# barlettacarmen/CrCNN

Hardware: AMD Instinct MI355X
Metric: encrypted images/sec (higher is better)
Workload: dtype u64

## Files before the change

crcnn_amd/csrc/kernels_mfma1.hip:

```cpp
#include "kernels.h"
#include "limbred.h"
#include "boxstage.h"
#include <cstdlib>

typedef int v4i __attribute__((ext_vector_type(4)));
typedef signed char i8;
#define NPL 7
#define MAXK 8

struct Conv1Args {
    const i8 *xr; const i8 *wl; u64 *ys; i8 *xl_out; const ModParams *mods; const u64 *bias;
    int n, k, B, Bout, b0, xd, yo, xs, ystr, P, F, mtiles;
    unsigned img_stride, plane_bytes, poly_bytes;
    unsigned out_img_bytes;
    int out_zdc;
    int narrow;
    int acc0[MAXK][13];
    u32 qbits[MAXK], qfold[MAXK];
    unsigned px_rs;
    int px_taps, px_yf, px_pair;
    int acc7[MAXK][7];
};

__device__ __forceinline__ void limb_digits1(u64 r, u64 q, int (&d)[NPL])
{
    long long v = r > (q >> 1) ? (long long)r - (long long)q : (long long)r;
#pragma unroll
    for (int l = 0; l < NPL; l++) { d[l] = (int)(signed char)(v & 0xff); v = (v - d[l]) >> 8; }
}

__device__ __forceinline__ void conv1_store4(const Conv1Args &a, i8 *stage, const long long (&cv)[4], int mm, int f0, int chan_bytes, u64 q, int slot, int b)
{
    if (mm >= 2 * a.P) return;
    if (a.xl_out) {
        if (f0 >= chan_bytes) return;
        u32 lo[4], hi[4];
#pragma unroll
        for (int reg = 0; reg < 4; reg++) { const u64 dg = f0 + reg < a.F ? centred_digit_bytes(cv[reg]) : 0; lo[reg] = (u32)dg;
            hi[reg] = (u32)(dg >> 32); }
        const u32 t0 = __builtin_amdgcn_perm(lo[1], lo[0], 0x05010400u), t1 = __builtin_amdgcn_perm(lo[1], lo[0], 0x07030602u);
        const u32 u0 = __builtin_amdgcn_perm(lo[3], lo[2], 0x05010400u), u1 = __builtin_amdgcn_perm(lo[3], lo[2], 0x07030602u);
        const u32 t2 = __builtin_amdgcn_perm(hi[1], hi[0], 0x05010400u), t3 = __builtin_amdgcn_perm(hi[1], hi[0], 0x07030602u);
        const u32 u2 = __builtin_amdgcn_perm(hi[3], hi[2], 0x05010400u), u3 = __builtin_amdgcn_perm(hi[3], hi[2], 0x07030602u);
        u32 pl[NPL];
        pl[0] = __builtin_amdgcn_perm(u0, t0, 0x05040100u); pl[1] = __builtin_amdgcn_perm(u0, t0, 0x07060302u);
        pl[2] = __builtin_amdgcn_perm(u1, t1, 0x05040100u); pl[3] = __builtin_amdgcn_perm(u1, t1, 0x07060302u);
        pl[4] = __builtin_amdgcn_perm(u2, t2, 0x05040100u); pl[5] = __builtin_amdgcn_perm(u2, t2, 0x07060302u);
        pl[6] = __builtin_amdgcn_perm(u3, t3, 0x05040100u);
        i8 *sp; unsigned pstride;
        if (a.out_zdc) { sp = stage + ((mm & 1) * a.P + (mm >> 1)) * a.out_zdc + f0; pstride = 2 * a.P * a.out_zdc; }
        else { sp = stage + mm * (NPL * 32) + f0; pstride = 32; }
#pragma unroll
        for (int l = 0; l < NPL; l++) *reinterpret_cast<u32 *>(sp + l * pstride) = pl[l];
    } else {
#pragma unroll
        for (int reg = 0; reg < 4; reg++)
            if (f0 + reg < a.F) a.ys[(((size_t)slot * a.B + b) * a.F + f0 + reg) * (2 * a.P) + mm] = (u64)(cv[reg] + ((cv[reg] >> 63) & (long long)q));
    }
}
__device__ __forceinline__ void conv1_copy_out(const Conv1Args &a, const i8 *stage, int slot, int b)
{
    i8 *dst = a.xl_out + ((size_t)slot * a.Bout + a.b0 + b) * a.out_img_bytes;
    if (a.out_zdc) {
        for (unsigned o = threadIdx.x; o < a.out_img_bytes / 16; o += blockDim.x)
            *reinterpret_cast<uint4 *>(dst + (size_t)o * 16) = *reinterpret_cast<const uint4 *>(stage + (size_t)o * 16);
    } else {
        const unsigned per_plane = a.out_img_bytes / (NPL * 16);
        for (unsigned o = threadIdx.x; o < NPL * per_plane; o += blockDim.x) {
            const unsigned l = o / per_plane, rem = o - l * per_plane;
            *reinterpret_cast<uint4 *>(dst + (size_t)o * 16) = *reinterpret_cast<const uint4 *>(stage + (rem >> 1) * (NPL * 32) + l * 32 +
                (rem & 1) * 16);
        }
    }
}

__global__ void __launch_bounds__(768) mfma_conv1_kernel(Conv1Args a)
{
    extern __shared__ __attribute__((aligned(16))) i8 lds[];
    const int lane = threadIdx.x & 63, wave = __builtin_amdgcn_readfirstlane(threadIdx.x >> 6), nwaves = blockDim.x >> 6;
    const int slot = blockIdx.x, i = slot / a.n, s = slot % a.n;
    const u64 q = a.mods[i].q;
    const u32 qbits = a.qbits[i], qfold = a.qfold[i];
    const int g = lane >> 4, r16 = lane & 15;
    const bool narrow = a.narrow != 0;
    const int nt = narrow ? (wave >> 2) & 1 : wave & 1;
    const int tile0 = !narrow ? wave >> 1 : nt ? wave - 4 : (wave < 4 ? wave : wave - 4), tile_step = !narrow ? nwaves >> 1 : nt ? 4 : nwaves - 4;
    const bool nar = narrow && nt;
    v4i wv[NPL];
    {
        const i8 *ws = a.wl + (size_t)slot * (NPL * 32 * 64) + (nt * 16 + r16) * 64 + g * 16;
        if (!nar) {
#pragma unroll
            for (int l = 0; l < NPL; l++) wv[l] = *reinterpret_cast<const v4i *>(ws + l * (32 * 64));
        } else {
            const i8 *wp = a.wl + (size_t)slot * (NPL * 32 * 64) + (16 + (r16 >> 2)) * 64 + g * 16;
#pragma unroll
            for (int grp = 0; grp < 2; grp++) {
                const int pl = 4 * grp + (r16 & 3);
                wv[grp] = pl < NPL ? *reinterpret_cast<const v4i *>(wp + pl * (32 * 64)) : v4i{0, 0, 0, 0};
            }
#pragma unroll
            for (int l = 2; l < NPL; l++) wv[l] = v4i{0, 0, 0, 0};
        }
    }
    u32 PB[7];
#pragma unroll
    for (int j = 0; j < 6; j++) PB[j] = (u32)a.acc0[i][2 * j] + ((u32)a.acc0[i][2 * j + 1] << 8);
    PB[6] = (u32)a.acc0[i][12];
    const u32 rcp_yo = (65536u + (u32)a.yo - 1) / (u32)a.yo;
    const int f0 = nt * 16 + 4 * g;
    long long bvc[4];
#pragma unroll
    for (int reg = 0; reg < 4; reg++) {
        const int f = f0 + reg;
        const u64 bv = (a.bias && f < a.F && !(lane & 1)) ? a.bias[((size_t)f * a.k + i) * a.n + s] : 0;
        bvc[reg] = bv > (q >> 1) ? (long long)(bv - q) : (long long)bv;
    }
    long long bvn = 0;
    if (nar) {
        const int f = 16 + g;
        const u64 bv = (a.bias && f < a.F && !(lane & 1)) ? a.bias[((size_t)f * a.k + i) * a.n + s] : 0;
        bvn = bv > (q >> 1) ? (long long)(bv - q) : (long long)bv;
    }
    i8 *stage = lds + 2 * (size_t)a.img_stride;
    const i8 *ximg = a.xr + (size_t)slot * a.B * a.img_stride;
    const int pieces = a.img_stride / 1024;
    auto issue_img = [&](int b) {
        i8 *dst = lds + (b & 1) * (size_t)a.img_stride;
        const i8 *src = ximg + (size_t)b * a.img_stride + lane * 16;
        for (int pc = wave; pc < pieces; pc += nwaves)
            __builtin_amdgcn_global_load_lds((const __attribute__((address_space(1))) void *)(src + pc * 1024),
                (__attribute__((address_space(3))) void *)(dst + pc * 1024), 16, 0, 0);
    };
    if (a.xl_out && a.out_zdc && threadIdx.x < 16) { const unsigned e = a.out_img_bytes - 16 + threadIdx.x;
        if (e >= (unsigned)(NPL * 2 * a.P * a.out_zdc)) stage[e] = 0; }
    issue_img(0);
    const int chan_bytes = a.out_zdc ? a.out_zdc : 32;
    for (int b = 0; b < a.B; b++) {
        __builtin_amdgcn_s_waitcnt(0 | (7 << 4) | (15 << 8));
        __syncthreads();
        if (b + 1 < a.B) issue_img(b + 1);
        const i8 *img = lds + (b & 1) * (size_t)a.img_stride;
        for (int mt = tile0; mt < a.mtiles; mt += tile_step) {
            v4i acc[13];
#pragma unroll
            for (int d = 0; d < 13; d++) acc[d] = v4i{0, 0, 0, 0};
            const int mm = mt * 16 + r16, mrow = min(mm, 2 * a.P - 1), p = mrow >> 1, c = mrow & 1, ox = (int)(((u32)p * rcp_yo) >> 16), oy = p - ox * a.yo;
            const int r0 = min(ox * a.xs + 2 * g, a.xd - 1), r1 = min(ox * a.xs + 2 * g + 1, a.xd - 1);
            const int off = oy * a.ystr, sh = off & 3;
            const i8 *p0 = img + c * a.poly_bytes + (off & ~3) + r0 * 32, *p1 = img + c * a.poly_bytes + (off & ~3) + r1 * 32;
            auto window = [&](int l) {
                const u32 *q0 = reinterpret_cast<const u32 *>(p0 + l * a.plane_bytes), *q1 = reinterpret_cast<const u32 *>(p1 + l * a.plane_bytes);
                const u32 a0 = q0[0], a1 = q0[1], a2 = q0[2], b0 = q1[0], b1 = q1[1], b2 = q1[2];
                return v4i{(int)__builtin_amdgcn_alignbyte(a1, a0, sh), (int)__builtin_amdgcn_alignbyte(a2, a1, sh), (int)__builtin_amdgcn_alignbyte(b1, b0,
                    sh),
                           (int)__builtin_amdgcn_alignbyte(b2, b1, sh)};
            };
            if (nar) {
                v4i hi6;
#pragma unroll
                for (int l = 0; l < NPL; l++) {
                    const v4i av = window(l);
                    acc[l] = __builtin_amdgcn_mfma_i32_16x16x64_i8(wv[0], av, v4i{0, 0, 0, 0}, 0, 0, 0);
                    if (l < 6) acc[7 + l] = __builtin_amdgcn_mfma_i32_16x16x64_i8(wv[1], av, v4i{0, 0, 0, 0}, 0, 0, 0);
                    else hi6 = __builtin_amdgcn_mfma_i32_16x16x64_i8(wv[1], av, v4i{0, 0, 0, 0}, 0, 0, 0);
                }
                int D[13];
#pragma unroll
                for (int d = 0; d < 13; d++) {
                    int sum = 0;
#pragma unroll
                    for (int l = 0; l < NPL; l++) {
                        const int m = d - l;
                        if (m < 0 || m >= NPL) continue;
                        sum += m < 4 ? acc[l][m] : (l < 6 ? acc[7 + l][m - 4] : hi6[m - 4]);
                    }
                    D[d] = sum;
                }
                const long long cvn = diag_fold_short_centred(D, q, qbits, qfold, bvn, PB);
                const int f = 16 + g;
                if (mm >= 2 * a.P) continue;
                if (a.xl_out) {
                    if (f >= chan_bytes) continue;
                    const u64 dg = f < a.F ? centred_digit_bytes(cvn) : 0;
                    i8 *sp; unsigned pstride;
                    if (a.out_zdc) { sp = stage + ((mm & 1) * a.P + (mm >> 1)) * a.out_zdc + f; pstride = 2 * a.P * a.out_zdc; }
                    else { sp = stage + mm * (NPL * 32) + f; pstride = 32; }
#pragma unroll
                    for (int l = 0; l < NPL; l++) sp[l * pstride] = (i8)(dg >> (8 * l));
                } else if (f < a.F) a.ys[(((size_t)slot * a.B + b) * a.F + f) * (2 * a.P) + mm] = (u64)(cvn + ((cvn >> 63) & (long long)q));
                continue;
            }
#pragma unroll
            for (int l = 0; l < NPL; l++) {
                const v4i av = window(l);
#pragma unroll
                for (int m2 = 0; m2 < NPL; m2++)
                    acc[l + m2] = __builtin_amdgcn_mfma_i32_16x16x64_i8(wv[m2], av, acc[l + m2], 0, 0, 0);
            }
            long long cv[4];
#pragma unroll
            for (int reg = 0; reg < 4; reg++) {
                int D[13];
#pragma unroll
                for (int d = 0; d < 13; d++) D[d] = acc[d][reg];
                cv[reg] = diag_fold_short_centred(D, q, qbits, qfold, bvc[reg], PB);
            }
            conv1_store4(a, stage, cv, mm, f0, chan_bytes, q, slot, b);
        }
        if (a.xl_out) {
            __syncthreads();
            conv1_copy_out(a, stage, slot, b);
        }
    }
}

#define NJ 5
__global__ void __launch_bounds__(512) mfma_conv1_kernel_px(Conv1Args a)
{
    extern __shared__ __attribute__((aligned(16))) i8 lds[];
    const int lane = threadIdx.x & 63, wave = __builtin_amdgcn_readfirstlane(threadIdx.x >> 6), nwaves = blockDim.x >> 6;
    const int slot = blockIdx.x, i = slot / a.n, s = slot % a.n;
    const u64 q = a.mods[i].q;
    const u32 qbits = a.qbits[i], qfold = a.qfold[i];
    const int g = lane >> 4, r16 = lane & 15, nt = wave & 1, tile0 = wave >> 1, tile_step = nwaves >> 1;
    v4i wv[NPL][NJ];
    {
        const i8 *ws = a.wl + (size_t)slot * (NPL * NJ * 32 * 64) + (nt * 16 + r16) * 64 + g * 16;
#pragma unroll
        for (int m = 0; m < NPL; m++)
#pragma unroll
            for (int j = 0; j < NJ; j++) wv[m][j] = *reinterpret_cast<const v4i *>(ws + (m * NJ + j) * (32 * 64));
    }
    u32 PB[4];
#pragma unroll
    for (int j = 0; j < 3; j++) PB[j] = (u32)a.acc7[i][2 * j] + ((u32)a.acc7[i][2 * j + 1] << 8);
    PB[3] = (u32)a.acc7[i][6];
    u32 toff[NJ];
#pragma unroll
    for (int j = 0; j < NJ; j++) {
        const int last = a.px_pair ? a.px_taps - 2 : a.px_taps - 1;
        const int t0 = min(2 * (4 * j + g), last), t1 = min(2 * (4 * j + g) + 1, a.px_taps - 1);
        const u32 o0 = (u32)(t0 / a.px_yf) * a.px_rs + (u32)(t0 % a.px_yf) * 8, o1 = (u32)(t1 / a.px_yf) * a.px_rs + (u32)(t1 % a.px_yf) * 8;
        toff[j] = o0 | (o1 << 16);
    }
    const u32 rcp_yo = (65536u + (u32)a.yo - 1) / (u32)a.yo;
    const int f0 = nt * 16 + 4 * g;
    long long bvc[4];
#pragma unroll
    for (int reg = 0; reg < 4; reg++) {
        const int f = f0 + reg;
        const u64 bv = (a.bias && f < a.F && !(lane & 1)) ? a.bias[((size_t)f * a.k + i) * a.n + s] : 0;
        bvc[reg] = bv > (q >> 1) ? (long long)(bv - q) : (long long)bv;
    }
    i8 *stage = lds + 2 * (size_t)a.img_stride;
    const i8 *ximg = a.xr + (size_t)slot * a.B * a.img_stride;
    const int pieces = a.img_stride / 1024;
    auto issue_img = [&](int b) {
        i8 *dst = lds + (b & 1) * (size_t)a.img_stride;
        const i8 *src = ximg + (size_t)b * a.img_stride + lane * 16;
        for (int pc = wave; pc < pieces; pc += nwaves)
            __builtin_amdgcn_global_load_lds((const __attribute__((address_space(1))) void *)(src + pc * 1024),
                (__attribute__((address_space(3))) void *)(dst + pc * 1024), 16, 0, 0);
    };
    if (a.xl_out && a.out_zdc && threadIdx.x < 16) { const unsigned e = a.out_img_bytes - 16 + threadIdx.x;
        if (e >= (unsigned)(NPL * 2 * a.P * a.out_zdc)) stage[e] = 0; }
    issue_img(0);
    const int chan_bytes = a.out_zdc ? a.out_zdc : 32;
    for (int b = 0; b < a.B; b++) {
        __builtin_amdgcn_s_waitcnt(0 | (7 << 4) | (15 << 8));
        __syncthreads();
        if (b + 1 < a.B) issue_img(b + 1);
        const i8 *img = lds + (b & 1) * (size_t)a.img_stride;
        for (int mt = tile0; mt < a.mtiles; mt += tile_step) {
            const int mm = mt * 16 + r16, mrow = min(mm, 2 * a.P - 1), p = mrow >> 1, c = mrow & 1, ox = (int)(((u32)p * rcp_yo) >> 16), oy = p - ox * a.yo;
            const i8 *win = img + c * a.poly_bytes + (u32)(ox * a.xs) * a.px_rs + (u32)(oy * a.ystr) * 8;
            v4i bv[NJ];
            if (a.px_pair) {
#pragma unroll
                for (int j = 0; j < NJ; j++) bv[j] = *reinterpret_cast<const v4i *>(win + (toff[j] & 0xffffu));
            } else {
#pragma unroll
                for (int j = 0; j < NJ; j++) {
                    const uint2 t0 = *reinterpret_cast<const uint2 *>(win + (toff[j] & 0xffffu)), t1 = *reinterpret_cast<const uint2 *>(win + (toff[j] >> 16));
                    bv[j] = v4i{(int)t0.x, (int)t0.y, (int)t1.x, (int)t1.y};
                }
            }
            v4i acc[NPL];
#pragma unroll
            for (int m = 0; m < NPL; m++) acc[m] = __builtin_amdgcn_mfma_i32_16x16x64_i8(wv[m][0], bv[0], v4i{0, 0, 0, 0}, 0, 0, 0);
#pragma unroll
            for (int j = 1; j < NJ; j++)
#pragma unroll
                for (int m = 0; m < NPL; m++) acc[m] = __builtin_amdgcn_mfma_i32_16x16x64_i8(wv[m][j], bv[j], acc[m], 0, 0, 0);
            long long cv[4];
#pragma unroll
            for (int reg = 0; reg < 4; reg++) {
                int E[NPL];
#pragma unroll
                for (int m = 0; m < NPL; m++) E[m] = acc[m][reg];
                cv[reg] = diag7_fold_centred(E, q, qbits, qfold, bvc[reg], PB);
            }
            conv1_store4(a, stage, cv, mm, f0, chan_bytes, q, slot, b);
        }
        if (a.xl_out) {
            __syncthreads();
            conv1_copy_out(a, stage, slot, b);
        }
    }
}

#define RG 4
#define RSL 32
__global__ void __launch_bounds__(256) limb_pack_rows1_kernel(const u64 *x, i8 *xr, const ModParams *mods, int n, int k, int B, int xd, int yd, int packed,
                                                              unsigned img_stride, unsigned plane_bytes, unsigned poly_bytes)
{
    __shared__ __attribute__((aligned(16))) i8 st[RSL * NPL * RG * 32];
    const int sblocks = n / RSL;
    const int sb = blockIdx.x % (sblocks * k), i = sb / sblocks, s0 = (sb % sblocks) * RSL;
    const int rgs = (xd + RG - 1) / RG;
    size_t r = blockIdx.x / (sblocks * k);
    const int rg = (int)(r % rgs); r /= rgs; const int c = (int)(r % 2); const int b = (int)(r / 2);
    const u64 q = mods[i].q;
    const int lane = threadIdx.x & (RSL - 1), qrow = (threadIdx.x >> 5) & (RG - 1), h = threadIdx.x >> 7, row = rg * RG + qrow;
    {
        u32 pl[NPL][4];
#pragma unroll
        for (int l = 0; l < NPL; l++)
#pragma unroll
            for (int wv = 0; wv < 4; wv++) pl[l][wv] = 0;
        if (row < xd) {
            const u64 *src = x + ((((size_t)b * xd * yd + (size_t)row * yd + h * 16) * 2 + c) * k + i) * (size_t)n + s0 + lane;
#pragma unroll
            for (int colx = 0; colx < 16; colx++)
                if (h * 16 + colx < yd) {
                    u64 v = src[(size_t)colx * 2 * k * n];
                    if (packed) v = (v & 0xffffffffULL) | ((v >> 32) << 28);
                    const u64 dg = balanced_digit_bytes(v, q);
#pragma unroll
                    for (int l = 0; l < NPL; l++) pl[l][colx >> 2] |= (u32)((dg >> (8 * l)) & 0xff) << (8 * (colx & 3));
                }
        }
        i8 *sp = st + (size_t)lane * (NPL * RG * 32) + qrow * 32 + h * 16;
#pragma unroll
        for (int l = 0; l < NPL; l++) *reinterpret_cast<uint4 *>(sp + l * (RG * 32)) = make_uint4(pl[l][0], pl[l][1], pl[l][2], pl[l][3]);
    }
    __syncthreads();
    const int pieces_per_run = RG * 2, rows_here = min(RG, xd - rg * RG);
    for (int o = threadIdx.x; o < RSL * NPL * pieces_per_run; o += 256) {
        const int run = o / pieces_per_run, part = o - run * pieces_per_run, sl = run / NPL, l = run - sl * NPL;
        if ((part >> 1) >= rows_here) continue;
        i8 *dst = xr + (((size_t)i * n + s0 + sl) * B + b) * img_stride + (size_t)l * plane_bytes + (size_t)c * poly_bytes + (size_t)(rg * RG) * 32 + part * 16;
        *reinterpret_cast<uint4 *>(dst) = *reinterpret_cast<const uint4 *>(st + (size_t)run * (RG * 32) + part * 16);
    }
}
template <bool BOX>
__global__ void __launch_bounds__(256) limb_pack_rows1_kernel_px(const u64 *x, i8 *xr, const ModParams *mods, int n, int k, int B, int xd, int yd, int packed,
                                                                 unsigned img_stride, unsigned poly_bytes, unsigned rs, int xdo, int ydo, int bxf, int byf, int xs,
                                                                 int ys)
{
    extern __shared__ __attribute__((aligned(16))) i8 stp[];
    const unsigned sstride = RG * rs + 16;
    const int sblocks = n / RSL;
    const int sb = blockIdx.x % (sblocks * k), i = sb / sblocks, s0 = (sb % sblocks) * RSL;
    const int rgs = (xdo + RG - 1) / RG;
    size_t r = blockIdx.x / (sblocks * k);
    const int rg = (int)(r % rgs); r /= rgs; const int c = (int)(r % 2); const int b = (int)(r / 2);
    const u64 q = mods[i].q;
    const int lane = threadIdx.x & (RSL - 1), qrow = (threadIdx.x >> 5) & (RG - 1), h = threadIdx.x >> 7, row = rg * RG + qrow;
    if (row < xdo) {
        const size_t cs = (size_t)2 * k * n;
        const u64 *src = x + ((((size_t)b * xd * yd + (size_t)row * yd + h * 16) * 2 + c) * k + i) * (size_t)n + s0 + lane;
        u64 *sp = reinterpret_cast<u64 *>(stp + (size_t)lane * sstride + qrow * rs) + h * 16;
        if constexpr (!BOX) {
#pragma unroll
            for (int colx = 0; colx < 16; colx++) {
                const int col = h * 16 + colx;
                if ((unsigned)col * 8 >= rs) continue;
                u64 dg = 0;
                if (col < yd) {
                    u64 v = src[(size_t)colx * cs];
                    if (packed) v = (v & 0xffffffffULL) | ((v >> 32) << 28);
                    dg = balanced_digit_bytes(v, q);
                }
                sp[colx] = dg;
            }
        } else {
            u64 sum[16];
#pragma unroll
            for (int colx = 0; colx < 16; colx++) sum[colx] = 0;
            for (int a = 0; a < bxf; a++)
                for (int bb = 0; bb < byf; bb++) {
                    const u64 *tp = src + ((size_t)a * xs * yd + (size_t)bb * ys) * cs;
#pragma unroll
                    for (int colx = 0; colx < 16; colx++)
                        if (h * 16 + colx < ydo) {
                            u64 v = tp[(size_t)colx * cs];
                            if (packed) v = (v & 0xffffffffULL) | ((v >> 32) << 28);
                            sum[colx] += v;
                        }
                }
#pragma unroll
            for (int colx = 0; colx < 16; colx++) {
                const int col = h * 16 + colx;
                if ((unsigned)col * 8 >= rs) continue;
                sp[colx] = col < ydo ? balanced_digit_bytes(sum_reduce16(sum[colx], q), q) : 0;
            }
        }
    }
    __syncthreads();
    const int per_run = RG * rs / 16, valid = min(RG, xdo - rg * RG) * (int)rs / 16;
    for (int o = threadIdx.x; o < RSL * per_run; o += 256) {
        const int sl = o / per_run, part = o - sl * per_run;
        if (part >= valid) continue;
        i8 *dst = xr + (((size_t)i * n + s0 + sl) * B + b) * img_stride + (size_t)c * poly_bytes + (size_t)(rg * RG) * rs + part * 16;
        *reinterpret_cast<uint4 *>(dst) = *reinterpret_cast<const uint4 *>(stp + (size_t)sl * sstride + part * 16);
    }
}
#define BOX_LD 16
static_assert(BOX_RG == RG && BOX_RSL == RSL, "boxstage.h describes this pack's workgroup");
__global__ void __launch_bounds__(256) limb_pack_box_kernel_px(const u64 *x, i8 *xr, const ModParams *mods, int n, int k, int B, int xd, int yd, int packed,
                                                               unsigned img_stride, unsigned poly_bytes, unsigned rs, int xdo, int ydo, int bxf, int byf, int xs,
                                                               int ys)
{
    extern __shared__ __attribute__((aligned(16))) i8 stp[];
    u64 *ring = reinterpret_cast<u64 *>(stp);
    i8 *dig = stp + box_ring_bytes(yd, bxf, xs);
    const unsigned sstride = RG * rs + 16;
    const int sblocks = n / RSL;
    const int sb = blockIdx.x % (sblocks * k), i = sb / sblocks, s0 = (sb % sblocks) * RSL;
    const int wpi = (int)(gridDim.x / (unsigned)(sblocks * k * 2 * B));
    size_t r = blockIdx.x / (sblocks * k);
    const int w = (int)(r % wpi); r /= wpi; const int c = (int)(r % 2); const int b = (int)(r / 2);
    const u64 q = mods[i].q;
    const int lane = threadIdx.x & (RSL - 1), seg = threadIdx.x >> 5, qrow = seg & (RG - 1), h = threadIdx.x >> 7;
    const u32 ring_px = box_ring_px(yd, bxf, xs);
    const size_t cs = (size_t)2 * k * n;
    const u64 *src = x + (((size_t)b * xd * yd * 2 + c) * k + i) * (size_t)n + s0 + lane;
    const int g0 = box_walk_first(w, xdo, wpi), g1 = box_walk_end(w, xdo, wpi);
    for (int g = g0; g < g1; g++) {
        const int p1 = box_load_end(g, xd, yd, bxf, xs);
        for (int pb = box_load_first(g, g == g0, xd, yd, bxf, xs) + seg; pb < p1; pb += 8 * BOX_LD) {
            u64 v[BOX_LD];
#pragma unroll
            for (int u = 0; u < BOX_LD; u++) v[u] = pb + 8 * u < p1 ? src[(size_t)(pb + 8 * u) * cs] : 0;
#pragma unroll
            for (int u = 0; u < BOX_LD; u++)
                if (pb + 8 * u < p1) {
                    u64 t = v[u];
                    if (packed) t = (t & 0xffffffffULL) | ((t >> 32) << 28);
                    ring[box_cell((u32)(pb + 8 * u), ring_px, lane)] = t;
                }
        }
        __syncthreads();
        const int row = g * RG + qrow;
        if (row < xdo) {
            u64 sum[16];
#pragma unroll
            for (int colx = 0; colx < 16; colx++) sum[colx] = 0;
            for (int a = 0; a < bxf; a++)
                for (int bb = 0; bb < byf; bb++) {
                    u32 pos = box_ring_pos(box_term_px(row, box_col(h, 0), a, bb, xs, ys, yd), ring_px);
#pragma unroll
                    for (int colx = 0; colx < 16; colx++) {
                        if (box_col(h, colx) < ydo) sum[colx] += ring[box_pos_cell(pos, lane)];
                        pos = box_ring_step(pos, 1, ring_px);
                    }
                }
            u64 *sp = reinterpret_cast<u64 *>(dig + (size_t)lane * sstride + qrow * rs) + h * 16;
#pragma unroll
            for (int colx = 0; colx < 16; colx++) {
                const int col = box_col(h, colx);
                if ((unsigned)col * 8 >= rs) continue;
                sp[colx] = col < ydo ? balanced_digit_bytes(sum_reduce16(sum[colx], q), q) : 0;
            }
        }
        __syncthreads();
        const int per_run = RG * rs / 16, valid = box_rows_here(g, xdo) * (int)rs / 16;
        for (int o = threadIdx.x; o < RSL * per_run; o += 256) {
            const int sl = o / per_run, part = o - sl * per_run;
            if (part >= valid) continue;
            i8 *dst = xr + (((size_t)i * n + s0 + sl) * B + b) * img_stride + (size_t)c * poly_bytes + (size_t)(g * RG) * rs + part * 16;
            *reinterpret_cast<uint4 *>(dst) = *reinterpret_cast<const uint4 *>(dig + (size_t)sl * sstride + part * 16);
        }
    }
}
__global__ void __launch_bounds__(64) limb_pack_w1_kernel(const u64 *w, i8 *wl, const ModParams *mods, int n, int k, int F, int xf, int yf)
{
    const int sblocks = n / 64;
    const int sb = blockIdx.x % (sblocks * k), i = sb / sblocks, s = (sb % sblocks) * 64 + threadIdx.x;
    size_t r = blockIdx.x / (sblocks * k);
    const int ky = (int)(r % yf); r /= yf; const int kx = (int)(r % xf); const int f = (int)(r / xf);
    const ModParams m = mods[i];
    int d[NPL]; limb_digits1(w[((((size_t)f * xf + kx) * yf + ky) * k + i) * (size_t)n + s], m.q, d);
    i8 *dst = wl + ((size_t)i * n + s) * (NPL * 32 * 64) + f * 64 + kx * 8 + ky;
#pragma unroll
    for (int l = 0; l < NPL; l++) dst[(size_t)l * (32 * 64)] = (i8)d[l];
}

__global__ void __launch_bounds__(64) limb_pack_w1_kernel_px(const u64 *w, i8 *wl, const ModParams *mods, int n, int k, int F, int xf, int yf)
{
    const int sblocks = n / 64;
    const int sb = blockIdx.x % (sblocks * k), i = sb / sblocks, s = (sb % sblocks) * 64 + threadIdx.x;
    size_t r = blockIdx.x / (sblocks * k);
    const int ky = (int)(r % yf); r /= yf; const int kx = (int)(r % xf); const int f = (int)(r / xf);
    const ModParams m = mods[i];
    u64 v = w[((((size_t)f * xf + kx) * yf + ky) * k + i) * (size_t)n + s];
    const int tap = kx * yf + ky, G = tap >> 1;
    i8 *dst = wl + ((size_t)i * n + s) * (NPL * NJ * 32 * 64) + ((G >> 2) * 32 + f) * 64 + (G & 3) * 16 + (tap & 1) * 8;
    for (int l = 0; l < NPL; l++) {
        int d[NPL]; limb_digits1(v, m.q, d);
#pragma unroll
        for (int dm = 0; dm < NPL; dm++) dst[(size_t)dm * (NJ * 32 * 64) + l] = (i8)d[dm];
        v = mulmod(v, 256, m);
    }
}

static inline unsigned conv1_poly_bytes(int xd) { return ((unsigned)xd + 1) * 32; }
static inline unsigned conv1_img_stride(int xd) { const unsigned b = NPL * 2 * conv1_poly_bytes(xd); return (b + 1023) / 1024 * 1024; }
static inline unsigned conv1_px_rs(int yd) { return ((unsigned)yd * 8 + 15) / 16 * 16; }
static inline unsigned conv1_px_poly_bytes(int xd, int yd) { const unsigned b = (unsigned)xd * conv1_px_rs(yd); return b + (128 + 256 - b % 256) % 256; }
static inline unsigned conv1_px_img_stride(int xd, int yd) { return (2 * conv1_px_poly_bytes(xd, yd) + 1023) / 1024 * 1024; }
static bool conv1_fits(unsigned img_stride, const Window &w)
{
    return 2 * (size_t)img_stride + (size_t)NPL * w.xo() * w.yo() * 2 * 32 <= 160 * 1024;
}
int k_limb_conv1_form(const crc_ctx *c, int xf, int yf, int nf)
{
    bool px = xf * yf <= 8 * NJ;
    for (int i = 0; i < c->k && px; i++) px = conv1_fold7_ok(c->tabs[i].m.q, c->tabs[i].m.bits, fold_constant(c->tabs[i].m.q, c->tabs[i].m.bits));
    const int forced = c->tune.conv1_form;
    if (forced == 1 || !px) return 1;
    if (forced == 2) return 2;
    return nf > 16 && nf <= 20 ? 1 : 2;
}
bool k_limb_conv1_shape(const crc_ctx *c, const LayerShape &s)
{
    const int xd = s.w.xd, yd = s.w.yd, xf = s.w.xf, yf = s.w.yf, nf = s.nf;
    if (s.zd != 1 || xf > 8 || yf > 8 || nf > 32 || yd > 32 || c->n < 64 || c->k > MAXK) return false;
    for (int i = 0; i < c->k; i++) if (!conv1_fold_ok(c->tabs[i].m.q, c->tabs[i].m.bits, fold_constant(c->tabs[i].m.q, c->tabs[i].m.bits))) return false;
    if (s.w.P() > 1024) return false;
    return conv1_fits(k_limb_conv1_form(c, xf, yf, nf) == 2 ? conv1_px_img_stride(xd, yd) : conv1_img_stride(xd), s.w);
}
bool k_limb_conv1_box_shape(const crc_ctx *c, const LayerShape &s, int bxf, int byf)
{
    if (bxf < 1 || byf < 1 || bxf * byf > 9) return false;
    const LayerShape sum{s.w.boxed(bxf, byf), s.zd, s.nf};
    if (sum.w.xd < sum.w.xf || sum.w.yd < sum.w.yf || !k_limb_conv1_shape(c, sum)) return false;
    return bxf * byf == 1 || k_limb_conv1_form(c, s.w.xf, s.w.yf, s.nf) == 2;
}
static size_t conv1_form_weights_bytes(const crc_ctx *c, int form) { return (size_t)c->n * c->k * NPL * 32 * 64 * (form == 2 ? NJ : 1); }
size_t k_limb_conv1_weights_bytes(const crc_ctx *c) { return conv1_form_weights_bytes(c, 2); }
size_t k_limb_conv1_weights_bytes_for(const crc_ctx *c, int nf, int xf, int yf) { return conv1_form_weights_bytes(c, k_limb_conv1_form(c, xf, yf, nf)); }
size_t k_limb_conv1_image_bytes(const crc_ctx *c, int B, const Window &w, int nf)
{
    return (size_t)c->n * c->k * B * (k_limb_conv1_form(c, w.xf, w.yf, nf) == 2 ? conv1_px_img_stride(w.xd, w.yd) : conv1_img_stride(w.xd));
}

static void conv1_tables(const crc_ctx *c, Conv1Args &a)
{
    for (int i = 0; i < c->k; i++) { conv1_bias_table(c->tabs[i].m.q, a.acc0[i]); conv1_bias7_table(c->tabs[i].m.q, a.acc7[i]); a.qbits[i] = c->tabs[i].m.bits;
        a.qfold[i] = fold_constant(c->tabs[i].m.q, c->tabs[i].m.bits); }
}

int k_limb_conv1_pack_weights(crc_ctx *c, const u64 *w, i8 *wl, int nf, int xf, int yf, hipStream_t st)
{
    const int form = k_limb_conv1_form(c, xf, yf, nf);
    HIPCHK(hipMemsetAsync(wl, 0, conv1_form_weights_bytes(c, form), st));
    const size_t blocks = (size_t)(c->n / 64) * c->k * nf * xf * yf;
    if (form == 2) hipLaunchKernelGGL(limb_pack_w1_kernel_px, dim3((unsigned)blocks), dim3(64), 0, st, w, wl, c->d_mods, c->n, c->k, nf, xf, yf);
    else hipLaunchKernelGGL(limb_pack_w1_kernel, dim3((unsigned)blocks), dim3(64), 0, st, w, wl, c->d_mods, c->n, c->k, nf, xf, yf);
    HIPCHK(hipGetLastError());
    return CRC_OK;
}
int k_limb_conv1(crc_ctx *c, const u64 *x, bool packed, i8 *xr, const i8 *wl, u64 *ys, i8 *xl_out, int Bout, int b0, const u64 *bias_ntt, int B, const Window &in,
                 int nf, hipStream_t st, int bxf, int byf)
{
    if (B == 0) return CRC_OK;
    if (!k_limb_conv1_box_shape(c, {in, 1, nf}, bxf, byf)) return CRC_ERR_UNSUPPORTED;
    const Window w = in.boxed(bxf, byf);
    const int xd = w.xd, yd = w.yd, xs = w.xs, xf = w.xf, yf = w.yf, xd_in = in.xd, yd_in = in.yd;
    const int form = k_limb_conv1_form(c, xf, yf, nf);
    Conv1Args a{};
    a.xr = xr; a.wl = wl; a.ys = ys; a.xl_out = xl_out; a.mods = c->d_mods; a.bias = bias_ntt;
    a.n = c->n; a.k = c->k; a.B = B; a.Bout = Bout; a.b0 = b0; a.xd = xd; a.yo = w.yo(); a.xs = xs; a.ystr = w.ys; a.P = w.P(); a.F = nf;
        a.mtiles = (2 * a.P + 15) / 16;
    a.out_zdc = a.P > 1 ? k_limb_flat_zdc(nf) : 0;
    a.out_img_bytes = a.out_zdc ? (unsigned)((NPL * 2 * a.P * a.out_zdc + 15) / 16 * 16) : (unsigned)(NPL * a.P * 2 * 32);
    conv1_tables(c, a);
    const size_t pack_blocks = (size_t)(c->n / RSL) * c->k * B * 2 * ((xd + RG - 1) / RG);
    if (pack_blocks > 0x7fffffffULL) return CRC_ERR_INVALID_ARGUMENT;
    if (form == 2) {
        a.px_rs = conv1_px_rs(yd); a.poly_bytes = conv1_px_poly_bytes(xd, yd); a.img_stride = conv1_px_img_stride(xd, yd);
        a.px_taps = xf * yf; a.px_yf = yf;
        a.px_pair = yf % 2 == 0 && w.ys % 2 == 0 ? 1 : 0;
        if (bxf * byf > 1 && box_staged(yd_in, bxf, xs, a.px_rs)) {
            const size_t lds = box_lds_bytes(yd_in, bxf, xs, a.px_rs);
            const int wpi = 1;
            { const int rc = crc_ctx_ensure_lds(c, (const void *)limb_pack_box_kernel_px, lds); if (rc) return rc; }
            hipLaunchKernelGGL(limb_pack_box_kernel_px, dim3((unsigned)((size_t)(c->n / RSL) * c->k * B * 2 * wpi)), dim3(256), lds, st, x, xr, c->d_mods, c->n,
                c->k, B, xd_in, yd_in, packed ? 1 : 0, a.img_stride, a.poly_bytes, a.px_rs, xd, yd, bxf, byf, xs, w.ys);
        } else if (bxf * byf > 1)
            hipLaunchKernelGGL(limb_pack_rows1_kernel_px<true>, dim3((unsigned)pack_blocks), dim3(256), RSL * (RG * a.px_rs + 16), st, x, xr, c->d_mods, c->n, c->k,
                B, xd_in, yd_in, packed ? 1 : 0, a.img_stride, a.poly_bytes, a.px_rs, xd, yd, bxf, byf, xs, w.ys);
        else
            hipLaunchKernelGGL(limb_pack_rows1_kernel_px<false>, dim3((unsigned)pack_blocks), dim3(256), RSL * (RG * a.px_rs + 16), st, x, xr, c->d_mods, c->n, c->k,
                B, xd_in, yd_in, packed ? 1 : 0, a.img_stride, a.poly_bytes, a.px_rs, xd, yd, 1, 1, xs, w.ys);
        HIPCHK(hipGetLastError());
        const size_t lds = 2 * (size_t)a.img_stride + (xl_out ? a.out_img_bytes : 0);
        { const int rc = crc_ctx_ensure_lds(c, (const void *)mfma_conv1_kernel_px, lds); if (rc) return rc; }
        hipLaunchKernelGGL(mfma_conv1_kernel_px, dim3((unsigned)(c->n * c->k)), dim3(64 * 8), lds, st, a);
        HIPCHK(hipGetLastError());
        return CRC_OK;
    }
    a.poly_bytes = conv1_poly_bytes(xd); a.plane_bytes = 2 * a.poly_bytes; a.img_stride = conv1_img_stride(xd);
    a.narrow = c->tune.conv1_narrow != 0 && nf > 16 && nf <= 20 ? 1 : 0;
    {
        hipLaunchKernelGGL(limb_pack_rows1_kernel, dim3((unsigned)pack_blocks), dim3(256), 0, st, x, xr, c->d_mods, c->n, c->k, B, xd, yd, packed ? 1 : 0,
            a.img_stride, a.plane_bytes, a.poly_bytes);
        HIPCHK(hipGetLastError());
    }
    auto busiest = [&](int nw) {
        int load[4] = {0, 0, 0, 0}, worst = 0;
        for (int w = 0; w < nw; w++) load[w & 3] += (a.mtiles - (w >> 1) + nw / 2 - 1) / (nw / 2);
        for (int sd = 0; sd < 4; sd++) worst = load[sd] > worst ? load[sd] : worst;
        return worst;
    };
    const int forced = c->tune.conv1_waves;
    const int nwaves = forced ? forced : a.narrow ? 12 : busiest(12) <= busiest(8) ? 12 : 8;
    const size_t lds = 2 * (size_t)a.img_stride + (xl_out ? a.out_img_bytes : 0);
    { const int rc = crc_ctx_ensure_lds(c, (const void *)mfma_conv1_kernel, lds); if (rc) return rc; }
    hipLaunchKernelGGL(mfma_conv1_kernel, dim3((unsigned)(c->n * c->k)), dim3(64 * nwaves), lds, st, a);
    HIPCHK(hipGetLastError());
    return CRC_OK;
}
```

Measured before the change: 817.2.

## Precompute conv1 row offsets in LDS and stage output plane-major

Adds a per-row table in LDS holding each output row's input-window offset and staging offset for the pixel-form conv1 kernel. The kernel prefetches the next tile's entry from this table instead of redoing the divide-by-reciprocal and offset math in the inner tile loop. The non-zdc staging buffer is now laid out plane-major, so the copy-out becomes a flat 16-byte copy with no per-element plane and remainder arithmetic. In exchange the kernel uses extra LDS for the table, and the fits check is widened to account for it.

```diff
diff --git a/crcnn_amd/csrc/conv1_rowtab.h b/crcnn_amd/csrc/conv1_rowtab.h
--- /dev/null
+++ b/crcnn_amd/csrc/conv1_rowtab.h
@@ -0,0 +1,27 @@
+#pragma once
+#include "modarith.h"
+
+#define CONV1_NPL 7
+
+struct Conv1RowGeom {
+    int P, yo, xs, ystr;
+    u32 px_rs, poly_bytes;
+    int zdc;
+};
+struct Conv1RowEntry { u32 win, stg; };
+
+CRC_HD int conv1_rowtab_rows(int P) { return (2 * P + 15) / 16 * 16; }
+CRC_HD size_t conv1_rowtab_bytes(int P) { return (size_t)conv1_rowtab_rows(P) * sizeof(Conv1RowEntry); }
+CRC_HD u32 conv1_stage_plane_stride(int P, int zdc) { return (u32)(2 * P) * (u32)(zdc ? zdc : 32); }
+CRC_HD u32 conv1_stage_bytes(int P, int zdc) { return zdc ? (CONV1_NPL * conv1_stage_plane_stride(P, zdc) + 15) / 16 * 16 : CONV1_NPL * conv1_stage_plane_stride(P, 0); }
+CRC_HD u32 conv1_stage_row(int mm, int P, int zdc) { return zdc ? (u32)((mm & 1) * P + (mm >> 1)) * (u32)zdc : (u32)mm * 32; }
+CRC_HD u32 conv1_window_row(int mm, const Conv1RowGeom &g)
+{
+    const u32 rcp_yo = (65536u + (u32)g.yo - 1) / (u32)g.yo;
+    const int mrow = mm < 2 * g.P - 1 ? mm : 2 * g.P - 1, p = mrow >> 1, c = mrow & 1, ox = (int)(((u32)p * rcp_yo) >> 16), oy = p - ox * g.yo;
+    return (u32)c * g.poly_bytes + (u32)(ox * g.xs) * g.px_rs + (u32)(oy * g.ystr) * 8;
+}
+CRC_HD Conv1RowEntry conv1_row_entry(int mm, const Conv1RowGeom &g)
+{
+    return Conv1RowEntry{conv1_window_row(mm, g), mm < 2 * g.P ? conv1_stage_row(mm, g.P, g.zdc) : 0u};
+}
diff --git a/crcnn_amd/csrc/kernels_mfma1.hip b/crcnn_amd/csrc/kernels_mfma1.hip
--- a/crcnn_amd/csrc/kernels_mfma1.hip
+++ b/crcnn_amd/csrc/kernels_mfma1.hip
@@ -1,9 +1,11 @@
 #include "kernels.h"
 #include "limbred.h"
 #include "boxstage.h"
+#include "conv1_rowtab.h"
 #include <cstdlib>
 
 typedef int v4i __attribute__((ext_vector_type(4)));
+typedef unsigned v2u __attribute__((ext_vector_type(2)));
 typedef signed char i8;
 #define NPL 7
 #define MAXK 8
@@ -29,7 +31,8 @@
     for (int l = 0; l < NPL; l++) { d[l] = (int)(signed char)(v & 0xff); v = (v - d[l]) >> 8; }
 }
 
-__device__ __forceinline__ void conv1_store4(const Conv1Args &a, i8 *stage, const long long (&cv)[4], int mm, int f0, int chan_bytes, u64 q, int slot, int b)
+__device__ __forceinline__ void conv1_store4(const Conv1Args &a, i8 *sp, unsigned pstride, const long long (&cv)[4], int mm, int f0, int chan_bytes, u64 q, int slot,
+                                             int b)
 {
     if (mm >= 2 * a.P) return;
     if (a.xl_out) {
@@ -47,9 +50,6 @@
         pl[2] = __builtin_amdgcn_perm(u1, t1, 0x05040100u); pl[3] = __builtin_amdgcn_perm(u1, t1, 0x07060302u);
         pl[4] = __builtin_amdgcn_perm(u2, t2, 0x05040100u); pl[5] = __builtin_amdgcn_perm(u2, t2, 0x07060302u);
         pl[6] = __builtin_amdgcn_perm(u3, t3, 0x05040100u);
-        i8 *sp; unsigned pstride;
-        if (a.out_zdc) { sp = stage + ((mm & 1) * a.P + (mm >> 1)) * a.out_zdc + f0; pstride = 2 * a.P * a.out_zdc; }
-        else { sp = stage + mm * (NPL * 32) + f0; pstride = 32; }
 #pragma unroll
         for (int l = 0; l < NPL; l++) *reinterpret_cast<u32 *>(sp + l * pstride) = pl[l];
     } else {
@@ -61,17 +61,8 @@
 __device__ __forceinline__ void conv1_copy_out(const Conv1Args &a, const i8 *stage, int slot, int b)
 {
     i8 *dst = a.xl_out + ((size_t)slot * a.Bout + a.b0 + b) * a.out_img_bytes;
-    if (a.out_zdc) {
-        for (unsigned o = threadIdx.x; o < a.out_img_bytes / 16; o += blockDim.x)
-            *reinterpret_cast<uint4 *>(dst + (size_t)o * 16) = *reinterpret_cast<const uint4 *>(stage + (size_t)o * 16);
-    } else {
-        const unsigned per_plane = a.out_img_bytes / (NPL * 16);
-        for (unsigned o = threadIdx.x; o < NPL * per_plane; o += blockDim.x) {
-            const unsigned l = o / per_plane, rem = o - l * per_plane;
-            *reinterpret_cast<uint4 *>(dst + (size_t)o * 16) = *reinterpret_cast<const uint4 *>(stage + (rem >> 1) * (NPL * 32) + l * 32 +
-                (rem & 1) * 16);
-        }
-    }
+    for (unsigned o = threadIdx.x * 16; o < a.out_img_bytes; o += blockDim.x * 16)
+        *reinterpret_cast<uint4 *>(dst + o) = *reinterpret_cast<const uint4 *>(stage + o);
 }
 
 __global__ void __launch_bounds__(768) mfma_conv1_kernel(Conv1Args a)
@@ -123,6 +114,148 @@
         bvn = bv > (q >> 1) ? (long long)(bv - q) : (long long)bv;
     }
     i8 *stage = lds + 2 * (size_t)a.img_stride;
+    const i8 *ximg = a.xr + (size_t)slot * a.B * a.img_stride;
+    const int pieces = a.img_stride / 1024;
+    auto issue_img = [&](int b) {
+        i8 *dst = lds + (b & 1) * (size_t)a.img_stride;
+        const i8 *src = ximg + (size_t)b * a.img_stride + lane * 16;
+        for (int pc = wave; pc < pieces; pc += nwaves)
+            __builtin_amdgcn_global_load_lds((const __attribute__((address_space(1))) void *)(src + pc * 1024),
+                (__attribute__((address_space(3))) void *)(dst + pc * 1024), 16, 0, 0);
+    };
+    if (a.xl_out && a.out_zdc && threadIdx.x < 16) { const unsigned e = a.out_img_bytes - 16 + threadIdx.x;
+        if (e >= (unsigned)(NPL * 2 * a.P * a.out_zdc)) stage[e] = 0; }
+    issue_img(0);
+    const int chan_bytes = a.out_zdc ? a.out_zdc : 32;
+    const unsigned pstride = conv1_stage_plane_stride(a.P, a.out_zdc);
+    for (int b = 0; b < a.B; b++) {
+        __builtin_amdgcn_s_waitcnt(0 | (7 << 4) | (15 << 8));
+        __syncthreads();
+        if (b + 1 < a.B) issue_img(b + 1);
+        const i8 *img = lds + (b & 1) * (size_t)a.img_stride;
+        for (int mt = tile0; mt < a.mtiles; mt += tile_step) {
+            v4i acc[13];
+#pragma unroll
+            for (int d = 0; d < 13; d++) acc[d] = v4i{0, 0, 0, 0};
+            const int mm = mt * 16 + r16, mrow = min(mm, 2 * a.P - 1), p = mrow >> 1, c = mrow & 1, ox = (int)(((u32)p * rcp_yo) >> 16), oy = p - ox * a.yo;
+            const int r0 = min(ox * a.xs + 2 * g, a.xd - 1), r1 = min(ox * a.xs + 2 * g + 1, a.xd - 1);
+            const int off = oy * a.ystr, sh = off & 3;
+            const i8 *p0 = img + c * a.poly_bytes + (off & ~3) + r0 * 32, *p1 = img + c * a.poly_bytes + (off & ~3) + r1 * 32;
+            auto window = [&](int l) {
+                const u32 *q0 = reinterpret_cast<const u32 *>(p0 + l * a.plane_bytes), *q1 = reinterpret_cast<const u32 *>(p1 + l * a.plane_bytes);
+                const u32 a0 = q0[0], a1 = q0[1], a2 = q0[2], b0 = q1[0], b1 = q1[1], b2 = q1[2];
+                return v4i{(int)__builtin_amdgcn_alignbyte(a1, a0, sh), (int)__builtin_amdgcn_alignbyte(a2, a1, sh), (int)__builtin_amdgcn_alignbyte(b1, b0,
+                    sh),
+                           (int)__builtin_amdgcn_alignbyte(b2, b1, sh)};
+            };
+            if (nar) {
+                v4i hi6;
+#pragma unroll
+                for (int l = 0; l < NPL; l++) {
+                    const v4i av = window(l);
+                    acc[l] = __builtin_amdgcn_mfma_i32_16x16x64_i8(wv[0], av, v4i{0, 0, 0, 0}, 0, 0, 0);
+                    if (l < 6) acc[7 + l] = __builtin_amdgcn_mfma_i32_16x16x64_i8(wv[1], av, v4i{0, 0, 0, 0}, 0, 0, 0);
+                    else hi6 = __builtin_amdgcn_mfma_i32_16x16x64_i8(wv[1], av, v4i{0, 0, 0, 0}, 0, 0, 0);
+                }
+                int D[13];
+#pragma unroll
+                for (int d = 0; d < 13; d++) {
+                    int sum = 0;
+#pragma unroll
+                    for (int l = 0; l < NPL; l++) {
+                        const int m = d - l;
+                        if (m < 0 || m >= NPL) continue;
+                        sum += m < 4 ? acc[l][m] : (l < 6 ? acc[7 + l][m - 4] : hi6[m - 4]);
+                    }
+                    D[d] = sum;
+                }
+                const long long cvn = diag_fold_short_centred(D, q, qbits, qfold, bvn, PB);
+                const int f = 16 + g;
+                if (mm >= 2 * a.P) continue;
+                if (a.xl_out) {
+                    if (f >= chan_bytes) continue;
+                    const u64 dg = f < a.F ? centred_digit_bytes(cvn) : 0;
+                    i8 *sp = stage + conv1_stage_row(mm, a.P, a.out_zdc) + f;
+#pragma unroll
+                    for (int l = 0; l < NPL; l++) sp[l * pstride] = (i8)(dg >> (8 * l));
+                } else if (f < a.F) a.ys[(((size_t)slot * a.B + b) * a.F + f) * (2 * a.P) + mm] = (u64)(cvn + ((cvn >> 63) & (long long)q));
+                continue;
+            }
+#pragma unroll
+            for (int l = 0; l < NPL; l++) {
+                const v4i av = window(l);
+#pragma unroll
+                for (int m2 = 0; m2 < NPL; m2++)
+                    acc[l + m2] = __builtin_amdgcn_mfma_i32_16x16x64_i8(wv[m2], av, acc[l + m2], 0, 0, 0);
+            }
+            long long cv[4];
+#pragma unroll
+            for (int reg = 0; reg < 4; reg++) {
+                int D[13];
+#pragma unroll
+                for (int d = 0; d < 13; d++) D[d] = acc[d][reg];
+                cv[reg] = diag_fold_short_centred(D, q, qbits, qfold, bvc[reg], PB);
+            }
+            conv1_store4(a, stage + conv1_stage_row(mm, a.P, a.out_zdc) + f0, pstride, cv, mm, f0, chan_bytes, q, slot, b);
+        }
+        if (a.xl_out) {
+            __syncthreads();
+            conv1_copy_out(a, stage, slot, b);
+        }
+    }
+}
+
+#define NJ 5
+__global__ void __launch_bounds__(512) mfma_conv1_kernel_px(Conv1Args a)
+{
+    extern __shared__ __attribute__((aligned(16))) i8 lds[];
+    const int lane = threadIdx.x & 63, wave = __builtin_amdgcn_readfirstlane(threadIdx.x >> 6), nwaves = blockDim.x >> 6;
+    const int slot = blockIdx.x, i = slot / a.n, s = slot % a.n;
+    const u64 q = a.mods[i].q;
+    const u32 qbits = a.qbits[i], qfold = a.qfold[i];
+    const int g = lane >> 4, r16 = lane & 15, nt = wave & 1, tile0 = wave >> 1, tile_step = nwaves >> 1;
+    v4i wv[NPL][NJ];
+    {
+        const i8 *ws = a.wl + (size_t)slot * (NPL * NJ * 32 * 64) + (nt * 16 + r16) * 64 + g * 16;
+#pragma unroll
+        for (int m = 0; m < NPL; m++)
+#pragma unroll
+            for (int j = 0; j < NJ; j++) wv[m][j] = *reinterpret_cast<const v4i *>(ws + (m * NJ + j) * (32 * 64));
+    }
+    u32 PB[4];
+#pragma unroll
+    for (int j = 0; j < 3; j++) PB[j] = (u32)a.acc7[i][2 * j] + ((u32)a.acc7[i][2 * j + 1] << 8);
+    PB[3] = (u32)a.acc7[i][6];
+    u32 toff[NJ];
+#pragma unroll
+    for (int j = 0; j < NJ; j++) {
+        const int last = a.px_pair ? a.px_taps - 2 : a.px_taps - 1;
+        const int t0 = min(2 * (4 * j + g), last), t1 = min(2 * (4 * j + g) + 1, a.px_taps - 1);
+        const u32 o0 = (u32)(t0 / a.px_yf) * a.px_rs + (u32)(t0 % a.px_yf) * 8, o1 = (u32)(t1 / a.px_yf) * a.px_rs + (u32)(t1 % a.px_yf) * 8;
+        toff[j] = o0 | (o1 << 16);
+    }
+    const int f0 = nt * 16 + 4 * g;
+    long long bvc[4];
+#pragma unroll
+    for (int reg = 0; reg < 4; reg++) {
+        const int f = f0 + reg;
+        const u64 bv = (a.bias && f < a.F && !(lane & 1)) ? a.bias[((size_t)f * a.k + i) * a.n + s] : 0;
+        bvc[reg] = bv > (q >> 1) ? (long long)(bv - q) : (long long)bv;
+    }
+    i8 *stage = lds + 2 * (size_t)a.img_stride;
+    const v2u *rowtab = reinterpret_cast<const v2u *>(stage + (a.xl_out ? a.out_img_bytes : 0));
+    {
+        const Conv1RowGeom geom{a.P, a.yo, a.xs, a.ystr, a.px_rs, a.poly_bytes, a.out_zdc};
+        for (int mm = threadIdx.x; mm < a.mtiles * 16; mm += blockDim.x) {
+            const Conv1RowEntry e = conv1_row_entry(mm, geom);
+            const_cast<v2u *>(rowtab)[mm] = v2u{e.win, e.stg};
+        }
+    }
+    const v2u *rowtab_lane = rowtab + r16;
+    __syncthreads();
+    v2u row = tile0 < a.mtiles ? rowtab_lane[tile0 * 16] : v2u{0u, 0u};
+    i8 *stage_lane = stage + f0;
+    const unsigned pstride = conv1_stage_plane_stride(a.P, a.out_zdc);
     const i8 *ximg = a.xr + (size_t)slot * a.B * a.img_stride;
     const int pieces = a.img_stride / 1024;
     auto issue_img = [&](int b) {
@@ -142,139 +275,9 @@
         if (b + 1 < a.B) issue_img(b + 1);
         const i8 *img = lds + (b & 1) * (size_t)a.img_stride;
         for (int mt = tile0; mt < a.mtiles; mt += tile_step) {
-            v4i acc[13];
-#pragma unroll
-            for (int d = 0; d < 13; d++) acc[d] = v4i{0, 0, 0, 0};
-            const int mm = mt * 16 + r16, mrow = min(mm, 2 * a.P - 1), p = mrow >> 1, c = mrow & 1, ox = (int)(((u32)p * rcp_yo) >> 16), oy = p - ox * a.yo;
-            const int r0 = min(ox * a.xs + 2 * g, a.xd - 1), r1 = min(ox * a.xs + 2 * g + 1, a.xd - 1);
-            const int off = oy * a.ystr, sh = off & 3;
-            const i8 *p0 = img + c * a.poly_bytes + (off & ~3) + r0 * 32, *p1 = img + c * a.poly_bytes + (off & ~3) + r1 * 32;
-            auto window = [&](int l) {
-                const u32 *q0 = reinterpret_cast<const u32 *>(p0 + l * a.plane_bytes), *q1 = reinterpret_cast<const u32 *>(p1 + l * a.plane_bytes);
-                const u32 a0 = q0[0], a1 = q0[1], a2 = q0[2], b0 = q1[0], b1 = q1[1], b2 = q1[2];
-                return v4i{(int)__builtin_amdgcn_alignbyte(a1, a0, sh), (int)__builtin_amdgcn_alignbyte(a2, a1, sh), (int)__builtin_amdgcn_alignbyte(b1, b0,
-                    sh),
-                           (int)__builtin_amdgcn_alignbyte(b2, b1, sh)};
-            };
-            if (nar) {
-                v4i hi6;
-#pragma unroll
-                for (int l = 0; l < NPL; l++) {
-                    const v4i av = window(l);
-                    acc[l] = __builtin_amdgcn_mfma_i32_16x16x64_i8(wv[0], av, v4i{0, 0, 0, 0}, 0, 0, 0);
-                    if (l < 6) acc[7 + l] = __builtin_amdgcn_mfma_i32_16x16x64_i8(wv[1], av, v4i{0, 0, 0, 0}, 0, 0, 0);
-                    else hi6 = __builtin_amdgcn_mfma_i32_16x16x64_i8(wv[1], av, v4i{0, 0, 0, 0}, 0, 0, 0);
-                }
-                int D[13];
-#pragma unroll
-                for (int d = 0; d < 13; d++) {
-                    int sum = 0;
-#pragma unroll
-                    for (int l = 0; l < NPL; l++) {
-                        const int m = d - l;
-                        if (m < 0 || m >= NPL) continue;
-                        sum += m < 4 ? acc[l][m] : (l < 6 ? acc[7 + l][m - 4] : hi6[m - 4]);
-                    }
-                    D[d] = sum;
-                }
-                const long long cvn = diag_fold_short_centred(D, q, qbits, qfold, bvn, PB);
-                const int f = 16 + g;
-                if (mm >= 2 * a.P) continue;
-                if (a.xl_out) {
-                    if (f >= chan_bytes) continue;
-                    const u64 dg = f < a.F ? centred_digit_bytes(cvn) : 0;
-                    i8 *sp; unsigned pstride;
-                    if (a.out_zdc) { sp = stage + ((mm & 1) * a.P + (mm >> 1)) * a.out_zdc + f; pstride = 2 * a.P * a.out_zdc; }
-                    else { sp = stage + mm * (NPL * 32) + f; pstride = 32; }
-#pragma unroll
-                    for (int l = 0; l < NPL; l++) sp[l * pstride] = (i8)(dg >> (8 * l));
-                } else if (f < a.F) a.ys[(((size_t)slot * a.B + b) * a.F + f) * (2 * a.P) + mm] = (u64)(cvn + ((cvn >> 63) & (long long)q));
-                continue;
-            }
-#pragma unroll
-            for (int l = 0; l < NPL; l++) {
-                const v4i av = window(l);
-#pragma unroll
-                for (int m2 = 0; m2 < NPL; m2++)
-                    acc[l + m2] = __builtin_amdgcn_mfma_i32_16x16x64_i8(wv[m2], av, acc[l + m2], 0, 0, 0);
-            }
-            long long cv[4];
-#pragma unroll
-            for (int reg = 0; reg < 4; reg++) {
-                int D[13];
-#pragma unroll
-                for (int d = 0; d < 13; d++) D[d] = acc[d][reg];
-                cv[reg] = diag_fold_short_centred(D, q, qbits, qfold, bvc[reg], PB);
-            }
-            conv1_store4(a, stage, cv, mm, f0, chan_bytes, q, slot, b);
-        }
-        if (a.xl_out) {
-            __syncthreads();
-            conv1_copy_out(a, stage, slot, b);
-        }
-    }
-}
-
-#define NJ 5
-__global__ void __launch_bounds__(512) mfma_conv1_kernel_px(Conv1Args a)
-{
-    extern __shared__ __attribute__((aligned(16))) i8 lds[];
-    const int lane = threadIdx.x & 63, wave = __builtin_amdgcn_readfirstlane(threadIdx.x >> 6), nwaves = blockDim.x >> 6;
-    const int slot = blockIdx.x, i = slot / a.n, s = slot % a.n;
-    const u64 q = a.mods[i].q;
-    const u32 qbits = a.qbits[i], qfold = a.qfold[i];
-    const int g = lane >> 4, r16 = lane & 15, nt = wave & 1, tile0 = wave >> 1, tile_step = nwaves >> 1;
-    v4i wv[NPL][NJ];
-    {
-        const i8 *ws = a.wl + (size_t)slot * (NPL * NJ * 32 * 64) + (nt * 16 + r16) * 64 + g * 16;
-#pragma unroll
-        for (int m = 0; m < NPL; m++)
-#pragma unroll
-            for (int j = 0; j < NJ; j++) wv[m][j] = *reinterpret_cast<const v4i *>(ws + (m * NJ + j) * (32 * 64));
-    }
-    u32 PB[4];
-#pragma unroll
-    for (int j = 0; j < 3; j++) PB[j] = (u32)a.acc7[i][2 * j] + ((u32)a.acc7[i][2 * j + 1] << 8);
-    PB[3] = (u32)a.acc7[i][6];
-    u32 toff[NJ];
-#pragma unroll
-    for (int j = 0; j < NJ; j++) {
-        const int last = a.px_pair ? a.px_taps - 2 : a.px_taps - 1;
-        const int t0 = min(2 * (4 * j + g), last), t1 = min(2 * (4 * j + g) + 1, a.px_taps - 1);
-        const u32 o0 = (u32)(t0 / a.px_yf) * a.px_rs + (u32)(t0 % a.px_yf) * 8, o1 = (u32)(t1 / a.px_yf) * a.px_rs + (u32)(t1 % a.px_yf) * 8;
-        toff[j] = o0 | (o1 << 16);
-    }
-    const u32 rcp_yo = (65536u + (u32)a.yo - 1) / (u32)a.yo;
-    const int f0 = nt * 16 + 4 * g;
-    long long bvc[4];
-#pragma unroll
-    for (int reg = 0; reg < 4; reg++) {
-        const int f = f0 + reg;
-        const u64 bv = (a.bias && f < a.F && !(lane & 1)) ? a.bias[((size_t)f * a.k + i) * a.n + s] : 0;
-        bvc[reg] = bv > (q >> 1) ? (long long)(bv - q) : (long long)bv;
-    }
-    i8 *stage = lds + 2 * (size_t)a.img_stride;
-    const i8 *ximg = a.xr + (size_t)slot * a.B * a.img_stride;
-    const int pieces = a.img_stride / 1024;
-    auto issue_img = [&](int b) {
-        i8 *dst = lds + (b & 1) * (size_t)a.img_stride;
-        const i8 *src = ximg + (size_t)b * a.img_stride + lane * 16;
-        for (int pc = wave; pc < pieces; pc += nwaves)
-            __builtin_amdgcn_global_load_lds((const __attribute__((address_space(1))) void *)(src + pc * 1024),
-                (__attribute__((address_space(3))) void *)(dst + pc * 1024), 16, 0, 0);
-    };
-    if (a.xl_out && a.out_zdc && threadIdx.x < 16) { const unsigned e = a.out_img_bytes - 16 + threadIdx.x;
-        if (e >= (unsigned)(NPL * 2 * a.P * a.out_zdc)) stage[e] = 0; }
-    issue_img(0);
-    const int chan_bytes = a.out_zdc ? a.out_zdc : 32;
-    for (int b = 0; b < a.B; b++) {
-        __builtin_amdgcn_s_waitcnt(0 | (7 << 4) | (15 << 8));
-        __syncthreads();
-        if (b + 1 < a.B) issue_img(b + 1);
-        const i8 *img = lds + (b & 1) * (size_t)a.img_stride;
-        for (int mt = tile0; mt < a.mtiles; mt += tile_step) {
-            const int mm = mt * 16 + r16, mrow = min(mm, 2 * a.P - 1), p = mrow >> 1, c = mrow & 1, ox = (int)(((u32)p * rcp_yo) >> 16), oy = p - ox * a.yo;
-            const i8 *win = img + c * a.poly_bytes + (u32)(ox * a.xs) * a.px_rs + (u32)(oy * a.ystr) * 8;
+            const int mm = mt * 16 + r16;
+            const v2u cur = row;
+            const i8 *win = img + cur.x;
             v4i bv[NJ];
             if (a.px_pair) {
 #pragma unroll
@@ -286,6 +289,7 @@
                     bv[j] = v4i{(int)t0.x, (int)t0.y, (int)t1.x, (int)t1.y};
                 }
             }
+            row = rowtab_lane[(mt + tile_step < a.mtiles ? mt + tile_step : tile0) * 16];
             v4i acc[NPL];
 #pragma unroll
             for (int m = 0; m < NPL; m++) acc[m] = __builtin_amdgcn_mfma_i32_16x16x64_i8(wv[m][0], bv[0], v4i{0, 0, 0, 0}, 0, 0, 0);
@@ -301,7 +305,7 @@
                 for (int m = 0; m < NPL; m++) E[m] = acc[m][reg];
                 cv[reg] = diag7_fold_centred(E, q, qbits, qfold, bvc[reg], PB);
             }
-            conv1_store4(a, stage, cv, mm, f0, chan_bytes, q, slot, b);
+            conv1_store4(a, stage_lane + cur.y, pstride, cv, mm, f0, chan_bytes, q, slot, b);
         }
         if (a.xl_out) {
             __syncthreads();
@@ -418,6 +422,7 @@
     }
 }
 #define BOX_LD 16
+static_assert(CONV1_NPL == NPL, "conv1_rowtab.h describes these kernels' digit planes");
 static_assert(BOX_RG == RG && BOX_RSL == RSL, "boxstage.h describes this pack's workgroup");
 __global__ void __launch_bounds__(256) limb_pack_box_kernel_px(const u64 *x, i8 *xr, const ModParams *mods, int n, int k, int B, int xd, int yd, int packed,
                                                                unsigned img_stride, unsigned poly_bytes, unsigned rs, int xdo, int ydo, int bxf, int byf, int xs,
@@ -521,9 +526,9 @@
 static inline unsigned conv1_px_rs(int yd) { return ((unsigned)yd * 8 + 15) / 16 * 16; }
 static inline unsigned conv1_px_poly_bytes(int xd, int yd) { const unsigned b = (unsigned)xd * conv1_px_rs(yd); return b + (128 + 256 - b % 256) % 256; }
 static inline unsigned conv1_px_img_stride(int xd, int yd) { return (2 * conv1_px_poly_bytes(xd, yd) + 1023) / 1024 * 1024; }
-static bool conv1_fits(unsigned img_stride, const Window &w)
-{
-    return 2 * (size_t)img_stride + (size_t)NPL * w.xo() * w.yo() * 2 * 32 <= 160 * 1024;
+static bool conv1_fits(unsigned img_stride, const Window &w, bool px)
+{
+    return 2 * (size_t)img_stride + (size_t)NPL * w.xo() * w.yo() * 2 * 32 + (px ? conv1_rowtab_bytes(w.xo() * w.yo()) : 0) <= 160 * 1024;
 }
 int k_limb_conv1_form(const crc_ctx *c, int xf, int yf, int nf)
 {
@@ -540,7 +545,8 @@
     if (s.zd != 1 || xf > 8 || yf > 8 || nf > 32 || yd > 32 || c->n < 64 || c->k > MAXK) return false;
     for (int i = 0; i < c->k; i++) if (!conv1_fold_ok(c->tabs[i].m.q, c->tabs[i].m.bits, fold_constant(c->tabs[i].m.q, c->tabs[i].m.bits))) return false;
     if (s.w.P() > 1024) return false;
-    return conv1_fits(k_limb_conv1_form(c, xf, yf, nf) == 2 ? conv1_px_img_stride(xd, yd) : conv1_img_stride(xd), s.w);
+    const bool px = k_limb_conv1_form(c, xf, yf, nf) == 2;
+    return conv1_fits(px ? conv1_px_img_stride(xd, yd) : conv1_img_stride(xd), s.w, px);
 }
 bool k_limb_conv1_box_shape(const crc_ctx *c, const LayerShape &s, int bxf, int byf)
 {
@@ -586,7 +592,7 @@
     a.n = c->n; a.k = c->k; a.B = B; a.Bout = Bout; a.b0 = b0; a.xd = xd; a.yo = w.yo(); a.xs = xs; a.ystr = w.ys; a.P = w.P(); a.F = nf;
         a.mtiles = (2 * a.P + 15) / 16;
     a.out_zdc = a.P > 1 ? k_limb_flat_zdc(nf) : 0;
-    a.out_img_bytes = a.out_zdc ? (unsigned)((NPL * 2 * a.P * a.out_zdc + 15) / 16 * 16) : (unsigned)(NPL * a.P * 2 * 32);
+    a.out_img_bytes = conv1_stage_bytes(a.P, a.out_zdc);
     conv1_tables(c, a);
     const size_t pack_blocks = (size_t)(c->n / RSL) * c->k * B * 2 * ((xd + RG - 1) / RG);
     if (pack_blocks > 0x7fffffffULL) return CRC_ERR_INVALID_ARGUMENT;
@@ -607,7 +613,7 @@
             hipLaunchKernelGGL(limb_pack_rows1_kernel_px<false>, dim3((unsigned)pack_blocks), dim3(256), RSL * (RG * a.px_rs + 16), st, x, xr, c->d_mods, c->n, c->k,
                 B, xd_in, yd_in, packed ? 1 : 0, a.img_stride, a.poly_bytes, a.px_rs, xd, yd, 1, 1, xs, w.ys);
         HIPCHK(hipGetLastError());
-        const size_t lds = 2 * (size_t)a.img_stride + (xl_out ? a.out_img_bytes : 0);
+        const size_t lds = 2 * (size_t)a.img_stride + (xl_out ? a.out_img_bytes : 0) + conv1_rowtab_bytes(a.P);
         { const int rc = crc_ctx_ensure_lds(c, (const void *)mfma_conv1_kernel_px, lds); if (rc) return rc; }
         hipLaunchKernelGGL(mfma_conv1_kernel_px, dim3((unsigned)(c->n * c->k)), dim3(64 * 8), lds, st, a);
         HIPCHK(hipGetLastError());
```

Result: faster. 828.0 (median of 6 runs) (+1.3%).
